# dcaustin33/intro_to_gaussian_splatting

Measured on AMD Instinct MI355X. Metric: Mpixels/sec forward raster (1M Gaussians, 1080p) + max |dpixel| vs CPU ref, higher is better.
Workload: dtype f32; 1 GPU; C3: synthetic 1M Gaussians, 1920x1080 (metric config); n_gaussians=1000000, width=1920, height=1080, tile=16, semantics=ref_cpu, layout=wh3, frames_in_flight=1, launch=one hipGraph replay per frame, frame_sync=speculative (GSX_FLAG_NO_SYNC), counts confirmed after the timed region, parallelism=1 GPU

## Files before the change

intro_to_gaussian_splatting_amd/csrc/gsx_blend.hip:

```cpp
#include <type_traits>

#include "gsx_internal.h"
#include "gsx_schedule_device.h"

namespace gsx {
namespace {

constexpr uint32_t kBatchCost = 5;
constexpr int kPad = 8, kSlots = 64 + kPad;
constexpr int kBlocks = 4;
struct __attribute__((aligned(16))) Staged {
    float4 rec[3][kSlots];
    uint16_t list[kBlocks][kSlots];
};

__device__ __forceinline__ uint32_t xcd_remap(uint32_t b, uint32_t n) {
    uint32_t xcd = b & 7u, i = b >> 3, q = n >> 3, r = n & 7u;
    uint32_t start = xcd < r ? xcd * (q + 1u) : r * (q + 1u) + (xcd - r) * q;
    return start + i;
}

__device__ __forceinline__ uint32_t scheduled_tile(uint32_t b, uint32_t nt, const uint32_t *__restrict__ sched) {
    if (!sched) return xcd_remap(b, nt);
    const uint32_t round = b >> 10, slot = b & 1023u;
    const uint32_t in_round = min(1024u, nt - (round << 10));
    return sched[(round << 10) + ((round & 1u) ? in_round - 1u - slot : slot)];
}

__device__ __forceinline__ uint32_t xcd_scheduled_tile(uint32_t b, uint32_t nt, uint32_t cap, const uint32_t *__restrict__ sched,
                                                       const uint32_t *__restrict__ header) {
    if (header[kHintSched] != nt) return b < nt ? xcd_remap(b, nt) : nt;
    const uint32_t x = b & 7u, i = b >> 3, mine = header[kHintXcdTiles + x];
    if (i >= mine) return nt;
    const uint32_t round = i >> 7, slot = i & 127u;
    const uint32_t in_round = min(128u, mine - (round << 7));
    return sched[(size_t)x * cap + (round << 7) + ((round & 1u) ? in_round - 1u - slot : slot)];
}


__device__ __forceinline__ void clear_block(uint32_t cb, const ClearPlan &cp, float *__restrict__ base) {
    int i = 0;
#pragma unroll
    for (int k = 1; k < 4; ++k) i = (k < cp.n && cb >= (uint32_t)cp.first[k]) ? k : i;
    const uint32_t per_row = (uint32_t)cp.fw[i] * 3u;
    const uint32_t total = (uint32_t)cp.rows[i] * per_row;
    const uint32_t e0 = (cb - (uint32_t)cp.first[i]) * (uint32_t)kClearFloats;
    const uint32_t e1 = min(total, e0 + (uint32_t)kClearFloats);
    float *origin = base + (int64_t)cp.s0[i] * cp.pitch + (int64_t)cp.f0[i] * 3;
    for (uint32_t e = e0 + threadIdx.x; e < e1; e += 64) {
        const uint32_t row = e / per_row, col = e - row * per_row;
        origin[(int64_t)row * cp.pitch + col] = 0.0f;
    }
}

__global__ void __launch_bounds__(64) clear_kernel(ClearPlan cp, float *__restrict__ base) {
    clear_block(blockIdx.x, cp, base);
}

constexpr float kRefOrderFlag = 2.0f;
enum { kKindSquare = 0, kKindMono = 1, kKindRefOrder = 2 };

struct Splat {
    float mx, c0, d1, h, r11, lop, cr, cg, cb, my;
    int kind;
    uint32_t blocks;
};

// ... 14 lines not shown
    }
}
__device__ __forceinline__ float exponent_y(const Splat &g, float p, float s0, float t0) {
    if (g.kind == kKindMono) {
        const float e_p = g.my - p;
        return __builtin_fmaf(e_p, __builtin_fmaf(e_p, g.r11, t0), s0);
    }
    const float w = __builtin_fmaf(-g.r11, p, t0);
    return __builtin_fmaf(-w, w, s0);
}

template <int NPX, bool WITH_REF = true>
__device__ __forceinline__ void composite(float px, const float (&e_p)[NPX], const Splat &g, float (&T)[NPX],
                                          float (&c0)[NPX], float (&c1)[NPX], float (&c2)[NPX], int blk, float ox, float oy) {
    float s0, t0;
    exponent_x(g, px, s0, t0);
    const bool kept = (g.blocks >> blk) & 1u;
    float ta[NPX], test[NPX];
#pragma unroll
    for (int j = 0; j < NPX; ++j) {
        float alpha = (WITH_REF && g.kind == kKindRefOrder)
                          ? alpha_ref(g.mx, g.c0, g.d1, g.h, g.r11, g.my, g.lop, ox + px, oy + e_p[j])
                          : __builtin_amdgcn_exp2f(exponent_y(g, e_p[j], s0, t0));
        alpha = kept ? alpha : 0.0f;
        ta[j] = T[j] * alpha;
        test[j] = T[j] - ta[j];
    }
    float m = test[0], tmin = T[0];
#pragma unroll
    for (int j = 1; j < NPX; ++j) {
        m = fminf(m, test[j]);
        tmin = fminf(tmin, T[j]);
    }
    if (__builtin_expect(__any((m < kStopRefCpu) | (tmin == 0.0f)), 0)) {
#pragma unroll
        for (int j = 0; j < NPX; ++j) {
            const bool stop = (T[j] == 0.0f) | (test[j] < kStopRefCpu);
            ta[j] = stop ? 0.0f : ta[j];
            test[j] = stop ? 0.0f : test[j];
        }
    }
#pragma unroll
    for (int j = 0; j < NPX; ++j) {
        c0[j] = __builtin_fmaf(ta[j], g.cr, c0[j]);
        c1[j] = __builtin_fmaf(ta[j], g.cg, c1[j]);
        c2[j] = __builtin_fmaf(ta[j], g.cb, c2[j]);
        T[j] = test[j];
    }
}

constexpr uint32_t kSkipBudget = 1u << 23;
enum { kBatchRegular = 0, kBatchWild = 1, kBatchMono = 2, kBatchRefOrder = 3, kBatchRefWild = 4, kBatchKindMask = 7, kBatchHasRef = 8 };
static_assert(kBatchMono < kBatchRefOrder, "the plain instances stop at kind >= kBatchRefOrder and composite a monomial-only batch");
enum { kStageWhole = 0, kStageBlocks = 1, kStageOneBlock = 2 };

__device__ __forceinline__ float skip_threshold(float bound, uint32_t &skipped, uint32_t budget) {
    const unsigned long long far1 = __ballot(bound < -26.0f), far2 = __ballot(bound < -33.0f), far3 = __ballot(bound < -40.0f);
    const uint32_t n3 = (uint32_t)__popcll(far3), n2 = (uint32_t)__popcll(far2) - n3, n1 = (uint32_t)__popcll(far1) - n2 - n3;
    const uint32_t cost3 = n3, cost23 = cost3 + (n2 << 7), cost123 = cost23 + (n1 << 14);
    if (skipped + cost123 <= budget) {
        skipped += cost123;
        return -26.0f;
    }
    if (skipped + cost23 <= budget) {
        skipped += cost23;
        return -33.0f;
    }
    if (skipped + cost3 <= budget) {
        skipped += cost3;
        return -40.0f;
    }
    return -__builtin_inff();
}

template <int MODE, bool WITH_REF = true>
__device__ __forceinline__ int stage_records(float4 a, float4 b, float4 c, bool have, uint32_t &nb, Staged &sh, int lane,
                                             float tile_x0, float tile_y0, float tile_side, uint32_t (&skipped)[kBlocks],
                                             uint32_t budget, int blk, uint32_t (&count)[kBlocks], uint32_t dead = 0u,
                                             unsigned long long *ref_slots = nullptr, const float4 *__restrict__ qraw = nullptr,
                                             uint32_t gi = 0u) {
    bool irregular = false, mono = false, refo = false;
    float bound[kBlocks] = {0.0f, 0.0f, 0.0f, 0.0f};
    float x_abs = 0.0f, y_abs = 0.0f;
    if (have) {
        refo = c.z == kRefOrderFlag;
        mono = !refo && c.z != 0.0f;
        if (WITH_REF) {
            x_abs = a.x;
            y_abs = a.y;
        }
        a.x -= tile_x0;
        a.y -= tile_y0;
        const bool bounded = !mono && a.z >= 0.0f;
        const float bx = a.x, by = a.y, bd1 = a.z, bh = a.w, br11 = b.x, blop = refo ? b.y + 0.02f : b.y;
        if (bounded) {
            auto over = [&](float x_lo, float x_hi, float y_lo, float y_hi) -> float {
                const float ex0 = bx - x_lo, ex1 = bx - x_hi;
                const float ey0 = by - y_lo, ey1 = by - y_hi;
                const float ex_min2 = ex0 * ex1 <= 0.0f ? 0.0f : fminf(ex0 * ex0, ex1 * ex1);
                const float w00 = __builtin_fmaf(br11, ey0, bh * ex0), w01 = __builtin_fmaf(br11, ey1, bh * ex0);
                const float w10 = __builtin_fmaf(br11, ey0, bh * ex1), w11 = __builtin_fmaf(br11, ey1, bh * ex1);
                const float wlo = fminf(fminf(w00, w01), fminf(w10, w11)), whi = fmaxf(fmaxf(w00, w01), fmaxf(w10, w11));
                const float wabs = fminf(fabsf(wlo), fabsf(whi));
                const float w_min2 = (wlo <= 0.0f && whi >= 0.0f) ? 0.0f : wabs * wabs;
                return blop - bd1 * ex_min2 - w_min2;
            };
            if (MODE == kStageWhole) {
                bound[0] = over(0.0f, tile_side - 1.0f, 0.0f, tile_side - 1.0f);
            } else if (MODE == kStageOneBlock) {
                bound[0] = over(8.0f * (float)(blk & 1), 8.0f * (float)(blk & 1) + 7.0f, 8.0f * (float)(blk >> 1), 8.0f * (float)(blk >> 1) + 7.0f);
            } else {
#pragma unroll
                for (int g = 0; g < kBlocks; ++g)
                    bound[g] = over(8.0f * (float)(g & 1), 8.0f * (float)(g & 1) + 7.0f, 8.0f * (float)(g >> 1), 8.0f * (float)(g >> 1) + 7.0f);
            }
            if (refo) {
                const float hi = tile_side - 1.0f;
                const float ex = fmaxf(fabsf(bx), fabsf(bx - hi)), ey = fmaxf(fabsf(by), fabsf(by - hi));
                const float S = 0.69314718f * ((bd1 + bh * bh) * (ex * ex) + 2.0f * fabsf(bh) * br11 * (ex * ey) + (br11 * br11) * (ey * ey));
                const float amax = __builtin_amdgcn_exp2f(fminf(over(0.0f, hi, 0.0f, hi), 0.0f));
                const float delta = 2.4e-7f * S;
                if (delta < 0.1f && delta * amax < 2e-5f) {
                    refo = false;
                    c.z = 0.0f;
                } else {
                    const float slack = 1.4427f * delta;
#pragma unroll
                    for (int g = 0; g < kBlocks; ++g) bound[g] += slack;
                }
            }
        }
        irregular = mono || refo || !(a.z >= 0.0f);
    }
    uint32_t bits = 0;
    unsigned long long kept_by[kBlocks] = {0ull, 0ull, 0ull, 0ull};
    if (MODE == kStageBlocks) {
#pragma unroll
        for (int g = 0; g < kBlocks; ++g) {
            if ((dead >> g) & 1u) continue;
            const float thr = skip_threshold(bound[g], skipped[g], budget);
            const bool k = have && !(bound[g] < thr);
            bits |= k ? (1u << g) : 0u;
            kept_by[g] = __ballot(k);
        }
    } else {
        const float thr = skip_threshold(bound[0], skipped[MODE == kStageOneBlock ? blk : 0], budget);
        bits = (have && !(bound[0] < thr)) ? 0xFu : 0u;
    }
    const bool keep = bits != 0u;
    float4 q4 = make_float4(0.f, 0.f, 0.f, 0.f);
    if (WITH_REF && refo && keep) q4 = qraw[gi];
    const unsigned long long mask = __ballot(keep);
    nb = (uint32_t)__popcll(mask);
    const uint32_t slot = __builtin_amdgcn_mbcnt_hi((uint32_t)(mask >> 32), __builtin_amdgcn_mbcnt_lo((uint32_t)mask, 0u));
    if (MODE == kStageBlocks) {
        const uint16_t null_slot = (uint16_t)(nb * 16u);
#pragma unroll
        for (int g = 0; g < kBlocks; ++g) {
            sh.list[g][lane] = null_slot;
            if (lane < kPad) sh.list[g][64 + lane] = null_slot;
        }
    }
    if (keep) {
        c.w = __uint_as_float(bits);
        if (WITH_REF && refo) {
            a = make_float4(x_abs, y_abs, q4.x, q4.y);
            b.x = q4.z;
            b.y = c.y;
            c.y = q4.w;
        } else {
            c.y = a.y;
            if (!mono) a.y = __builtin_fmaf(b.x, a.y, a.w * a.x);
        }
        sh.rec[0][slot] = a;
        sh.rec[1][slot] = b;
        sh.rec[2][slot] = c;
        if (MODE == kStageBlocks) {
#pragma unroll
            for (int g = 0; g < kBlocks; ++g)
                if ((bits >> g) & 1u)
                    sh.list[g][__builtin_amdgcn_mbcnt_hi((uint32_t)(kept_by[g] >> 32), __builtin_amdgcn_mbcnt_lo((uint32_t)kept_by[g], 0u))] = (uint16_t)(slot * 16u);
        }
    }
    if (MODE == kStageBlocks) {
#pragma unroll
        for (int g = 0; g < kBlocks; ++g) count[g] = (uint32_t)__popcll(kept_by[g]);
    }
    if (lane < kPad) {
        sh.rec[0][nb + lane] = make_float4(0.0f, 0.0f, 0.0f, 0.0f);
        sh.rec[1][nb + lane] = make_float4(0.0f, -__builtin_inff(), 0.0f, 0.0f);
        sh.rec[2][nb + lane] = make_float4(0.0f, 0.0f, 0.0f, __uint_as_float(0xFu));
    }
    unsigned long long ref_lanes = __ballot(refo && keep), in_slots = 0ull;
    while (ref_lanes) {
        const int l = __builtin_ctzll(ref_lanes);
        ref_lanes &= ref_lanes - 1ull;
        in_slots |= 1ull << __popcll(mask & ((1ull << l) - 1ull));
    }
    if (ref_slots) *ref_slots = in_slots;
    const int kind = (__any(mono && keep) && (WITH_REF || !in_slots))
                         ? kBatchMono
                         : (in_slots ? ((WITH_REF && __any(irregular && !refo && keep)) ? kBatchRefWild : kBatchRefOrder)
                                     : (__any(irregular && keep) ? kBatchWild : kBatchRegular));
    return kind | ((WITH_REF && in_slots) ? kBatchHasRef : 0);
}

template <int MODE, bool WITH_REF = true>
__device__ __forceinline__ int stage_batch(const Record *__restrict__ rec, const float4 *__restrict__ qraw,
                                           const uint32_t *__restrict__ vals,
                                           uint32_t base, uint32_t &nb, Staged &sh, int lane, float tile_x0,
                                           float tile_y0, float tile_side, uint32_t (&skipped)[kBlocks], uint32_t (&count)[kBlocks],
                                           uint32_t budget = kSkipBudget, const uint32_t *idx = nullptr, int blk = 0,
                                           uint32_t dead = 0u, unsigned long long *ref_slots = nullptr) {
    float4 a = make_float4(0.f, 0.f, 0.f, 0.f), b = a, c = a;
    const bool have = (uint32_t)lane < nb;
    uint32_t gi = 0u;
    if (have) {
        gi = idx ? *idx : vals[base + lane];
        const Record *q = rec + gi;
        a = q->a;
        b = q->b;
        c = q->c;
    }
    return stage_records<MODE, WITH_REF>(a, b, c, have, nb, sh, lane, tile_x0, tile_y0, tile_side, skipped, budget, blk, count, dead,
                                         ref_slots, qraw, gi);
}

typedef float v2f __attribute__((ext_vector_type(2)));

__device__ __forceinline__ v2f pk_fma(v2f a, v2f b, v2f c) { return __builtin_elementwise_fma(a, b, c); }
__device__ __forceinline__ v2f pk_exp2(v2f p) { return v2f{__builtin_amdgcn_exp2f(p.x), __builtin_amdgcn_exp2f(p.y)}; }
__device__ __forceinline__ v2f splat2(float v) { return v2f{v, v}; }

__device__ __forceinline__ void alphas(float4 A, float r11, float lop, float cx, v2f cya, v2f cyb, v2f &al_a,
                                       v2f &al_b) {
    const float e_x = A.x - cx;
    const float s0 = __builtin_fmaf(-(A.z * e_x), e_x, lop);
    const float c = __builtin_fmaf(-A.w, cx, A.y);
    const v2f wa = pk_fma(splat2(-r11), cya, splat2(c)), wb = pk_fma(splat2(-r11), cyb, splat2(c));
    al_a = pk_exp2(pk_fma(-wa, wa, splat2(s0)));
    al_b = pk_exp2(pk_fma(-wb, wb, splat2(s0)));
}

__device__ __forceinline__ void alphas_mono(float4 A, float yp, float q11, float lop, float cx, v2f cya, v2f cyb, v2f &al_a,
                                            v2f &al_b) {
    const float e_x = A.x - cx;
    const float s0 = __builtin_fmaf(e_x * e_x, A.z, lop);
    const float t0 = e_x * A.w;
    const v2f ea = splat2(yp) - cya, eb = splat2(yp) - cyb;
    al_a = pk_exp2(pk_fma(ea, pk_fma(ea, splat2(q11), splat2(t0)), splat2(s0)));
    al_b = pk_exp2(pk_fma(eb, pk_fma(eb, splat2(q11), splat2(t0)), splat2(s0)));
}

__device__ __forceinline__ void alphas_ref(float4 A, float q10, float q11, float op, float fx, v2f fya, v2f fyb, v2f &al_a,
                                           v2f &al_b) {
    const float e0 = A.x - fx, d0 = -0.5f * e0;
    const float p00 = d0 * A.z, p01 = d0 * A.w;
    const v2f e1a = splat2(A.y) - fya, e1b = splat2(A.y) - fyb;
    const v2f d1a = splat2(-0.5f) * e1a, d1b = splat2(-0.5f) * e1b;
    const v2f t0a = pk_fma(d1a, splat2(q10), splat2(p00)), t0b = pk_fma(d1b, splat2(q10), splat2(p00));
    const v2f t1a = pk_fma(d1a, splat2(q11), splat2(p01)), t1b = pk_fma(d1b, splat2(q11), splat2(p01));
    const v2f pa = t0a * splat2(e0) + t1a * e1a, pb = t0b * splat2(e0) + t1b * e1b;
    const float l2e = 1.44269504088896340736f;
    al_a = pk_exp2(pa * splat2(l2e)) * splat2(op);
    al_b = pk_exp2(pb * splat2(l2e)) * splat2(op);
}

#define GSX_ACCUMULATE(ta_a, ta_b, cr, cg, cb)          \
    do {                                                \
        c0a = pk_fma(ta_a, splat2(cr), c0a);            \
        c1a = pk_fma(ta_a, splat2(cg), c1a);            \
        c2a = pk_fma(ta_a, splat2(cb), c2a);            \
        c0b = pk_fma(ta_b, splat2(cr), c0b);            \
        c1b = pk_fma(ta_b, splat2(cg), c1b);            \
        c2b = pk_fma(ta_b, splat2(cb), c2b);            \
    } while (0)

__device__ __forceinline__ void checked_pair(v2f alpha, v2f &T, v2f &ta) {
// ... 127 lines not shown
                    const float w = __builtin_fmaf(-Bq.x, cy, __builtin_fmaf(-A.w, cx, A.y));
                    alpha[u] = __builtin_amdgcn_exp2f(__builtin_fmaf(-w, w, s0));
                }
                float ta[kTrip], Tt = T;
                if (!checked) {
                    float m = T;
#pragma unroll
                    for (int u = 0; u < kTrip; ++u) {
                        ta[u] = Tt * alpha[u];
                        Tt = Tt - ta[u];
                        m = fminf(m, Tt);
                    }
                    if (__builtin_expect(__any(!(m >= kStopRefCpu)), 0)) {
                        checked = true;
                        Tt = T;
                    }
                }
                if (checked) {
#pragma unroll
                    for (int u = 0; u < kTrip; ++u) {
                        const float t_a = Tt * alpha[u], t = Tt - t_a;
                        const bool stop = (Tt == 0.0f) | (t < kStopRefCpu);
                        ta[u] = stop ? 0.0f : t_a;
                        Tt = stop ? 0.0f : t;
                    }
                }
#pragma unroll
                for (int u = 0; u < kTrip; ++u) {
                    const float2 rg_ = *reinterpret_cast<const float2 *>(&sh.rec[1][k + u].z);
                    const float cb = sh.rec[2][k + u].x;
                    c0 = __builtin_fmaf(ta[u], rg_.x, c0);
                    c1 = __builtin_fmaf(ta[u], rg_.y, c1);
                    c2 = __builtin_fmaf(ta[u], cb, c2);
                }
                T = Tt;
            }
        }
        tile_sync<REF>();
        if (__ballot(T > 0.0f) == 0ull) break;
    }
    if (cost_out && lane == 0) atomicMax(cost_out, cost | 0x80000000u);
    if (REF && saw_ref && lane == 0 && redo) atomicAdd(redo, 1u);
    float *o = out.ptr + (int64_t)(px - out.x0) * out.stride_x + (int64_t)(py - out.y0) * out.stride_y;
    o[0] = c0;
    o[1] = c1;
    o[2] = c2;
}

template <bool REF>
__device__ __forceinline__ void blend_tile16(const Record *__restrict__ rec, const float4 *__restrict__ qraw,
                                             const uint32_t *__restrict__ vals,
                                             const uint2 *__restrict__ ranges, const TileGrid &g, const OutDesc &out,
                                             const LongTiles &lt, uint32_t budget, const BlendHints &hints, const TileSpan &span,
                                             uint32_t t, Staged &sh) {
    const int lane = REF ? (int)(threadIdx.x & 63u) : (int)threadIdx.x;
    const int tx = g.wx0 + (int)(t / (uint32_t)g.nwy()), ty = g.wy0 + (int)(t % (uint32_t)g.nwy());
    if ((span.axis ? ty : tx) < span.lo || (span.axis ? ty : tx) >= span.hi) return;
    const bool y_contig = out.stride_y < out.stride_x;
    const int lx = y_contig ? (lane >> 2) : (lane & 15);
    const int ly0 = 4 * (y_contig ? (lane & 3) : (lane >> 4));
    const int px = tx * 16 + lx, py0 = ty * 16 + ly0;
    const float cx = (float)lx;
    float cy[4];
#pragma unroll
    for (int j = 0; j < 4; ++j) cy[j] = (float)(ly0 + j);
    const v2f cya = v2f{cy[0], cy[1]}, cyb = v2f{cy[2], cy[3]};
    const int blk = (lx >> 3) | ((ly0 >> 3) << 1);
    const uint16_t *my_list = sh.list[blk];
    const char *rec_a = reinterpret_cast<const char *>(&sh.rec[0][0]), *rec_b = reinterpret_cast<const char *>(&sh.rec[1][0]),
               *rec_c = reinterpret_cast<const char *>(&sh.rec[2][0]);

    float T[4] = {1.0f, 1.0f, 1.0f, 1.0f};
    float c0[4] = {0, 0, 0, 0}, c1[4] = {0, 0, 0, 0}, c2[4] = {0, 0, 0, 0};
    v2f Ta = splat2(1.0f), Tb = splat2(1.0f);
    v2f c0a = splat2(0.0f), c1a = c0a, c2a = c0a, c0b = c0a, c1b = c0a, c2b = c0a;

    bool checked = false;
    bool restart_scalar = false;
    uint2 rg = ranges[t];
    rg.x = (uint32_t)__builtin_amdgcn_readfirstlane((int)rg.x);
    rg.y = (uint32_t)__builtin_amdgcn_readfirstlane((int)rg.y);
    if (hints.lens && lane == 0 && t == 0) {
        const bool by_cost = hints.header[kHintLens] == (uint32_t)g.count() && hints.header[kHintSched] == (uint32_t)g.count();
        hints.header[kHintLens] = (uint32_t)g.count();
        if (lt.max && by_cost) {
            const uint32_t found = *lt.count, pct = max(hints.header[kHintLongPct], lt.cost_pct);
            hints.header[kHintLongPct] = found > 192u ? min(pct + pct / 4u, 1000u) : (found < 64u ? max(pct - pct / 8u, lt.cost_pct) : pct);
        }
    }
    if (rg.y & kLongFlag) return;
    bool saw_ref = false;
    uint32_t cost = 0;
    uint32_t skipped[kBlocks] = {0u, 0u, 0u, 0u};
    unsigned long long lanes_of[kBlocks];
#pragma unroll
    for (int gb = 0; gb < kBlocks; ++gb) lanes_of[gb] = __ballot(blk == gb);
    uint32_t dead = 0u;
    uint32_t idx = rg.x + (uint32_t)lane < rg.y ? vals[rg.x + lane] : 0u;
    for (uint32_t base = rg.x; base < rg.y; base += 64) {
        uint32_t nb = (uint32_t)__builtin_amdgcn_readfirstlane((int)min(64u, rg.y - base));
        const uint32_t idx_now = idx;
        if (base + 64u + (uint32_t)lane < rg.y) idx = vals[base + 64u + lane];
        uint32_t count[kBlocks];
        unsigned long long ref_slots = 0ull;
        const int kind_all = stage_batch<kStageBlocks, REF>(rec, qraw, vals, base, nb, sh, lane, (float)(tx * 16), (float)(ty * 16),
                                                            16.0f, skipped, count, budget, &idx_now, 0, dead, &ref_slots);
        const int kind = kind_all & kBatchKindMask;
        const bool wild = kind != kBatchRegular;
        if (REF && (kind_all & kBatchHasRef)) saw_ref = true;
        const uint32_t nl = max(max(count[0], count[1]), max(count[2], count[3]));
        cost += nl + kBatchCost;
        tile_sync<REF>();
        if (!REF && kind >= kBatchRefOrder) {
            if (lane == 0) atomicAdd(lt.redo, 1u);
            return;
        } else if (kind == kBatchMono) {
            restart_scalar = true;
            break;
        } else {
            constexpr int kTrip = 4;
            uint32_t k = 0;
            auto trip = [&](auto n_tag) __attribute__((always_inline)) -> bool {
                constexpr int N = decltype(n_tag)::value;
                v2f ta_a[N], ta_b[N], ta = Ta, tb = Tb;
                uint32_t slot[N];
#pragma unroll
                for (int u = 0; u < N; ++u) {
                    slot[u] = my_list[k + u];
                    const float4 A = *reinterpret_cast<const float4 *>(rec_a + slot[u]);
                    const float2 Bq = *reinterpret_cast<const float2 *>(rec_b + slot[u]);
                    v2f aa, ab;
                    alphas(A, Bq.x, Bq.y, cx, cya, cyb, aa, ab);
                    ta_a[u] = ta * aa;
                    ta_b[u] = tb * ab;
                    ta = ta - ta_a[u];
                    tb = tb - ta_b[u];
                }
                if (__builtin_expect(__any(!(min4(ta, tb) >= kStopRefCpu)), 0)) return false;
#pragma unroll
                for (int u = 0; u < N; ++u) {
                    const float2 rg_ = *reinterpret_cast<const float2 *>(rec_b + slot[u] + 8);
                    const float cb = *reinterpret_cast<const float *>(rec_c + slot[u]);
                    GSX_ACCUMULATE(ta_a[u], ta_b[u], rg_.x, rg_.y, cb);
                }
                Ta = ta;
                Tb = tb;
                k += N;
                return true;
            };
            auto exact_pair = [&]() __attribute__((always_inline)) {
                const uint32_t s0_ = my_list[k], s1_ = my_list[k + 1];
// ... 9 lines not shown
                checked_pair(aa1, Ta, ta1a);
                checked_pair(ab1, Tb, ta1b);
                GSX_ACCUMULATE(ta1a, ta1b, B1.z, B1.w, cb1);
                k += 2;
            };
            if (!wild) {
                while (!checked && k + kTrip <= nl) checked = !trip(std::integral_constant<int, kTrip>());
                while (!checked && k < nl) checked = !trip(std::integral_constant<int, 2>());
            }
            if (!REF || kind < kBatchRefOrder) {
                while (k < nl) exact_pair();
            } else {
                const float fx_ = (float)(tx * 16) + cx;
                const v2f fya = splat2((float)(ty * 16)) + cya, fyb = splat2((float)(ty * 16)) + cyb;
                auto is_ref = [&](uint32_t s_) -> bool { return (s_ >> 4) < 64u && ((ref_slots >> (s_ >> 4)) & 1ull) != 0ull; };
                while (k < nl) {
                    if (kind == kBatchRefOrder && !checked && k + kTrip <= nl) {
                        bool flagged = false;
#pragma unroll
                        for (int u = 0; u < kTrip; ++u) flagged |= is_ref(my_list[k + u]);
                        if (!__any(flagged)) {
                            checked = !trip(std::integral_constant<int, kTrip>());
                            continue;
                        }
                    }
                    const uint32_t s0_ = my_list[k], s1_ = my_list[k + 1];
                    const bool r0 = is_ref(s0_), r1 = is_ref(s1_);
                    if (!__any(r0 | r1)) {
                        exact_pair();
                        continue;
                    }
                    const float4 A0 = *reinterpret_cast<const float4 *>(rec_a + s0_), B0 = *reinterpret_cast<const float4 *>(rec_b + s0_);
                    const float2 C0 = *reinterpret_cast<const float2 *>(rec_c + s0_);
                    v2f aa, ab, ta_a, ta_b;
                    if (r0)
                        alphas_ref(A0, B0.x, C0.y, B0.y, fx_, fya, fyb, aa, ab);
                    else
                        alphas(A0, B0.x, B0.y, cx, cya, cyb, aa, ab);
                    checked_pair(aa, Ta, ta_a);
                    checked_pair(ab, Tb, ta_b);
                    GSX_ACCUMULATE(ta_a, ta_b, B0.z, B0.w, C0.x);
                    k += 1;
                }
            }
        }
        tile_sync<REF>();
        const unsigned long long alive = __ballot((Ta.x > 0.0f) | (Ta.y > 0.0f) | (Tb.x > 0.0f) | (Tb.y > 0.0f));
        if (alive == 0ull) break;
        if (checked) {
#pragma unroll
            for (int gb = 0; gb < kBlocks; ++gb) dead |= (alive & lanes_of[gb]) == 0ull ? (1u << gb) : 0u;
        }
    }
    if (restart_scalar) {
        tile_sync<REF>();
#pragma unroll
        for (int j = 0; j < 4; ++j) {
            T[j] = 1.0f;
            c0[j] = c1[j] = c2[j] = 0.0f;
        }
#pragma unroll
        for (int gb = 0; gb < kBlocks; ++gb) skipped[gb] = 0u;
        for (uint32_t base = rg.x; base < rg.y; base += 64) {
            uint32_t nb = (uint32_t)__builtin_amdgcn_readfirstlane((int)min(64u, rg.y - base));
            uint32_t count[kBlocks];
            const int later = stage_batch<kStageBlocks, REF>(rec, qraw, vals, base, nb, sh, lane, (float)(tx * 16), (float)(ty * 16),
                                                             16.0f, skipped, count, budget);
            if (REF && (later & kBatchHasRef)) saw_ref = true;
            if (!REF && (later & kBatchKindMask) >= kBatchRefOrder) {
                if (lane == 0) atomicAdd(lt.redo, 1u);
                return;
            }
            cost += 4u * nb;
            tile_sync<REF>();
            for (uint32_t k = 0; k < nb; ++k) {
                const Splat s = read_splat(sh, k);
                composite<4, REF>(cx, cy, s, T, c0, c1, c2, blk, (float)(tx * 16), (float)(ty * 16));
            }
            tile_sync<REF>();
            if (__ballot((T[0] > 0.0f) | (T[1] > 0.0f) | (T[2] > 0.0f) | (T[3] > 0.0f)) == 0ull) break;
        }
    } else {
        c0[0] = c0a.x; c0[1] = c0a.y; c0[2] = c0b.x; c0[3] = c0b.y;
        c1[0] = c1a.x; c1[1] = c1a.y; c1[2] = c1b.x; c1[3] = c1b.y;
        c2[0] = c2a.x; c2[1] = c2a.y; c2[2] = c2b.x; c2[3] = c2b.y;
    }

    if (hints.lens && lane == 0) hints.lens[t] = cost;
    if (REF && saw_ref && lane == 0 && lt.redo) atomicAdd(lt.redo, 1u);
    float *o = out.ptr + (int64_t)(px - out.x0) * out.stride_x + (int64_t)(py0 - out.y0) * out.stride_y;
    if (y_contig && (reinterpret_cast<uintptr_t>(o) & 15u) == 0) {
        float4 *o4 = reinterpret_cast<float4 *>(o);
        o4[0] = make_float4(c0[0], c1[0], c2[0], c0[1]);
        o4[1] = make_float4(c1[1], c2[1], c0[2], c1[2]);
        o4[2] = make_float4(c2[2], c0[3], c1[3], c2[3]);
    } else {
#pragma unroll
        for (int j = 0; j < 4; ++j) {
            float *oj = o + (int64_t)j * out.stride_y;
            oj[0] = c0[j];
            oj[1] = c1[j];
            oj[2] = c2[j];
        }
    }
}

template <bool REF>
__device__ __forceinline__ void blend_tile16_grid(const Record *__restrict__ rec, const float4 *__restrict__ qraw,
                                                  const uint32_t *__restrict__ vals, const uint2 *__restrict__ ranges,
                                                  const TileGrid &g, const OutDesc &out, const ClearPlan &cp, const LongTiles &lt,
                                                  uint32_t nhelpers, const uint32_t *__restrict__ sched, uint32_t budget,
                                                  const BlendHints &hints, uint32_t tile_blocks, uint32_t sched_cap_,
                                                  const TileSpan &span, Staged &sh) {
    const uint32_t nrank = hints.samples ? kRankGroups : 0u;
    const uint32_t rank0 = hints.rank_last ? gridDim.x - nrank : 0u;
    if (blockIdx.x - rank0 < nrank) {
        if (span.first) rank_samples(blockIdx.x - rank0, (int)threadIdx.x, hints);
        return;
    }
    const uint32_t block = hints.rank_last ? blockIdx.x : blockIdx.x - nrank;
    if (block < nhelpers) {
        const uint32_t b = block, slot = (b >> 5) * 8u + (b & 7u);
        const int quarter = (int)((b >> 3) & 3u);
        if (slot >= min(*lt.count, lt.max)) return;
        const uint32_t lt_tile = lt.list[slot];
        {
            const int lead = span.axis ? g.wy0 + (int)(lt_tile % (uint32_t)g.nwy()) : g.wx0 + (int)(lt_tile / (uint32_t)g.nwy());
            if (lead < span.lo || lead >= span.hi) return;
        }
        blend_long_tile_quarter<REF>(rec, qraw, vals, ranges, g, out, lt_tile, quarter, sh, budget,
                                     hints.lens ? hints.lens + lt_tile : nullptr, lt.redo);
        return;
    }
    const uint32_t bid = block - nhelpers;
    if (bid >= tile_blocks) {
        if (span.first) clear_block(bid - tile_blocks, cp, out.ptr);
        return;
    }
    const uint32_t t = hints.xcd_sched ? xcd_scheduled_tile(bid, (uint32_t)g.count(), sched_cap_, sched, hints.header)
                                       : scheduled_tile(bid, (uint32_t)g.count(), sched);
    if (t >= (uint32_t)g.count()) return;
    blend_tile16<REF>(rec, qraw, vals, ranges, g, out, lt, budget, hints, span, t, sh);
}

#ifndef GSX_PLAIN_WAVES
#define GSX_PLAIN_WAVES 8
#endif
__global__ void __launch_bounds__(64) __attribute__((amdgpu_waves_per_eu(GSX_PLAIN_WAVES, 8)))
    blend_tile16_kernel(const Record *__restrict__ rec, const float4 *__restrict__ qraw, const uint32_t *__restrict__ vals,
                        const uint2 *__restrict__ ranges, TileGrid g, OutDesc out, ClearPlan cp, LongTiles lt,
                        uint32_t nhelpers, const uint32_t *__restrict__ sched, uint32_t budget, BlendHints hints,
                        uint32_t tile_blocks, uint32_t sched_cap_, TileSpan span) {
    __shared__ Staged sh;
    blend_tile16_grid<false>(rec, qraw, vals, ranges, g, out, cp, lt, nhelpers, sched, budget, hints, tile_blocks, sched_cap_, span, sh);
}

#ifndef GSX_REF_WAVES
#define GSX_REF_WAVES 4
#endif
__global__ void __launch_bounds__(64) __attribute__((amdgpu_waves_per_eu(GSX_REF_WAVES, 8)))
    blend_tile16_ref_kernel(const Record *__restrict__ rec, const float4 *__restrict__ qraw, const uint32_t *__restrict__ vals,
                            const uint2 *__restrict__ ranges, TileGrid g, OutDesc out, ClearPlan cp, LongTiles lt,
                            uint32_t nhelpers, const uint32_t *__restrict__ sched, uint32_t budget, BlendHints hints,
                            uint32_t tile_blocks, uint32_t sched_cap_, TileSpan span) {
    __shared__ Staged sh;
    blend_tile16_grid<true>(rec, qraw, vals, ranges, g, out, cp, lt, nhelpers, sched, budget, hints, tile_blocks, sched_cap_, span, sh);
}

__global__ void __launch_bounds__(64)
    blend_generic_kernel(const Record *__restrict__ rec, const float4 *__restrict__ qraw, const uint32_t *__restrict__ vals,
                         const uint2 *__restrict__ ranges, TileGrid g, OutDesc out, ClearPlan cp) {
    __shared__ Staged sh;
    if (blockIdx.x >= (uint32_t)g.count()) {
        clear_block(blockIdx.x - (uint32_t)g.count(), cp, out.ptr);
        return;
    }
    const int lane = threadIdx.x;
    const uint32_t t = xcd_remap(blockIdx.x, (uint32_t)g.count());
    const int tx = g.wx0 + (int)(t / (uint32_t)g.nwy()), ty = g.wy0 + (int)(t % (uint32_t)g.nwy());
    const int Ts = g.tile, npx = Ts * Ts;
    const uint2 rg = ranges[t];
    const bool fast_y = out.stride_y < out.stride_x;
    const bool blocks = Ts == 16;
    for (int chunk = 0; chunk < npx; chunk += 64) {
        uint32_t skipped[kBlocks] = {0u, 0u, 0u, 0u}, count[kBlocks];
        const int p = chunk + lane;
        const bool valid = p < npx;
        const int pf = p % Ts, ps = p / Ts;
        const int lx = fast_y ? ps : pf, ly = fast_y ? pf : ps;
        const int px = tx * Ts + lx, py = ty * Ts + ly;
        const float fx = (float)lx, fy = (float)ly;
        const int blk = blocks ? ((lx >> 3) | ((ly >> 3) << 1)) & 3 : 0;
        float T[1] = {1.0f}, c0[1] = {0.0f}, c1[1] = {0.0f}, c2[1] = {0.0f};
        for (uint32_t base = rg.x; base < rg.y; base += 64) {
            uint32_t nb = min(64u, rg.y - base);
            if (blocks)
                (void)stage_batch<kStageBlocks>(rec, qraw, vals, base, nb, sh, lane, (float)(tx * Ts), (float)(ty * Ts), (float)Ts, skipped, count);
            else
                (void)stage_batch<kStageWhole>(rec, qraw, vals, base, nb, sh, lane, (float)(tx * Ts), (float)(ty * Ts), (float)Ts, skipped, count);
            __syncthreads();
            for (uint32_t k = 0; k < nb; ++k) {
                const Splat s = read_splat(sh, k);
                const float e_p[1] = {fy};
                composite<1>(fx, e_p, s, T, c0, c1, c2, blk, (float)(tx * Ts), (float)(ty * Ts));
            }
            __syncthreads();
            if (__ballot(valid && T[0] > 0.0f) == 0ull) break;
        }
        if (valid) {
            float *o = out.ptr + (int64_t)(px - out.x0) * out.stride_x + (int64_t)(py - out.y0) * out.stride_y;
            o[0] = c0[0];
            o[1] = c1[0];
            o[2] = c2[0];
        }
    }
}

constexpr float kStdAlphaMin = 1.0f / 255.0f, kStdStop = 0.0001f;
// ... 314 lines not shown
```

intro_to_gaussian_splatting_amd/gaussian_scene.py:

```python
from __future__ import annotations

import ctypes
from collections import OrderedDict
from typing import Dict, Optional, Sequence, Tuple

import torch

from . import _ffi
from .colmap import read_camera_file, read_image_file
from .gaussians import Gaussians
from .image import GaussianImage
from .schema import PreprocessedScene


def _ptr(t: Optional[torch.Tensor]):
    return ctypes.c_void_p(0 if t is None else t.data_ptr())


def _check_f32(name: str, t: torch.Tensor, device: torch.device) -> torch.Tensor:
    if t.dtype != torch.float32:
        raise TypeError("%s must be float32, got %s" % (name, t.dtype))
    if t.device != device:
        raise ValueError("%s is on %s, expected %s" % (name, t.device, device))
    return t if t.is_contiguous() else t.contiguous()
# ... 578 lines not shown
            dev = g.points.device
            _require_gpu(dev)
            n = int(g.points.shape[0])
            k = (int(g.sh_degree) + 1) ** 2
            pts = _check_f32("points", g.points.detach().reshape(n, 3), dev)
            sh = _check_f32("sh", g.sh.detach().reshape(n, k, 3), dev)
            gc = _check_f32("grad_colors", grad_colors.detach().reshape(n, 3), dev)
            gsh = torch.empty((n, k, 3), dtype=torch.float32, device=dev)
            gview = torch.empty((n, 3), dtype=torch.float32, device=dev) if with_points else None
            center = (ctypes.c_float * 3)(*self.images[image_idx].camera_center_host)
            with torch.cuda.device(dev):
                rc = lib.gsx_sh_backward(_ptr(pts), _ptr(sh), int(g.sh_degree), n, center, _ptr(gc), _ptr(gsh), _ptr(gview),
                                         _stream_handle(dev))
            _ffi.check(rc)
        return gsh, gview

    def _note_count(self, cap_key, n_instances: int, n_kept: int = 0, n_redo: Optional[int] = None) -> None:
        self._instances_hint = max(self._instances_hint, int(n_instances * 1.1))
        self._cap_hints[cap_key] = int(n_instances * 1.1) + 4096
        self._kept_hints[cap_key] = max(1, int(n_kept))
        if n_redo is not None:
            self._n_redo_seen[cap_key] = int(n_redo)
        if cap_key[2] is None and cap_key[3] == "ref_cpu":
            self._last_instances = n_instances

    def _ensure_pinned_pool(self) -> None:
        if self._pinned_pool is None:
            self._pinned_pool = torch.zeros((_PINNED_SLOTS, ctypes.sizeof(_ffi.GsxFrameStats)),
                                            dtype=torch.uint8).pin_memory()

    def _pinned_slot(self) -> torch.Tensor:
        self._ensure_pinned_pool()
        slot = self._pinned_pool[self._pinned_next % _PINNED_SLOTS]
        self._pinned_next += 1
        slot.zero_()
        return slot

    def confirm_frames(self) -> int:
        if not self._pending:
            return 0
        torch.cuda.synchronize(self.gaussians.points.device)
        redone = 0
        pending, self._pending = self._pending, []
        for pinned, cap_key, ran_plain, call in pending:
            st = ctypes.cast(ctypes.c_void_p(pinned.data_ptr()), ctypes.POINTER(_ffi.GsxFrameStats)).contents
            self._note_count(cap_key, int(st.n_instances), int(st.n_kept), int(st.n_redo))
            if st.n_instances > st.reserved or (ran_plain and st.n_redo > 0):
                redone += 1
                self.render_image_hip(**call)
        return redone

    def capture_frame(self, image_idx: int, tile_size: int = 16, layout: str = "wh3",
                      semantics: str = "ref_cpu", movable_camera: bool = False,
                      headroom: float = 1.1) -> "CapturedFrame":
        if _wants_grad(self.gaussians):
            _refuse_with_grad("capture_frame")
        dev = self.gaussians.points.device
        _require_gpu(dev)
        cam = self.images[image_idx].gsx_camera()
        shape = (cam.width, cam.height, 3) if layout == "wh3" else (cam.height, cam.width, 3)
        out = torch.empty(shape, dtype=torch.float32, device=dev)
        cam_buf = None
        if movable_camera:
            cam_buf = torch.frombuffer(bytearray(bytes(cam)), dtype=torch.uint8).to(dev)
        kw = dict(tile_size=tile_size, layout=layout, out=out, semantics=semantics, camera_buffer=cam_buf)
        st = {}
        self.render_image_hip(image_idx, stats=st, **kw)
        lib = _ffi.load()
        n = int(self.gaussians.points.shape[0])
        cap = int(st["n_instances"] * max(float(headroom), 1.0)) + 4096
        nbytes = lib.gsx_workspace_bytes(n, cam.width, cam.height, tile_size, cap)
        if nbytes == 0:
            raise _ffi.GsxError(_ffi.GSX_ERR_INVALID_ARGUMENT, "gsx_workspace_bytes rejected the sizes")
        private = dict(cap=cap, workspace=torch.empty(nbytes, dtype=torch.uint8, device=dev), kept=int(st["n_kept"]),
                       rows_flag=0 if semantics == "std_3dgs" else _ffi.rows_flag(n, int(st["n_visible"])),
                       plain=(not movable_camera) and int(st.get("n_redo", 1)) == 0 and
                       int(st.get("n_tiles", 0)) >= _PLAIN_MIN_TILES,
                       pinned=torch.zeros(ctypes.sizeof(_ffi.GsxFrameStats), dtype=torch.uint8).pin_memory(), inputs=[],
                       hints=[torch.zeros(lib.gsx_hints_bytes(cam.width, cam.height, tile_size), dtype=torch.uint8,
                                          device=dev), False])
        stream = torch.cuda.Stream(dev)
        with torch.cuda.stream(stream):
            self.render_image_hip(image_idx, _private=private, **kw)
        torch.cuda.synchronize(dev)
        graph = torch.cuda.CUDAGraph()
        with torch.cuda.graph(graph, stream=stream):
            self.render_image_hip(image_idx, no_sync=True, _private=private, **kw)
        call = dict(image_idx=image_idx, **kw)
        frame = CapturedFrame(self, graph, out, private["pinned"], call, camera_buffer=cam_buf,
                              workspace=private["workspace"], capacity=cap, inputs=private["inputs"])
        frame._hints = private["hints"][0]
        frame._plain_footprints = bool(private["plain"])
        return frame

    def render_image(self, image_idx: int, tile_size: int = 16, geometry_gradients: bool = False) -> torch.Tensor:
        frame = self.render_image_hip(image_idx, tile_size=tile_size, layout="wh3", geometry_gradients=geometry_gradients)
        host = torch.empty(frame.shape, dtype=frame.dtype, pin_memory=True)
        host.copy_(frame, non_blocking=True)
        torch.cuda.current_stream(frame.device).synchronize()
        return host

    render = render_image

    def render_images(self, image_indices, tile_size: int = 16):
        if _wants_grad(self.gaussians):
            _refuse_with_grad("render_images")
        dev = self.gaussians.points.device
        _require_gpu(dev)
        copy_stream = torch.cuda.Stream(dev)
        frames, hosts, copied, checks, pending = [None, None], [None, None], [None, None], [None, None], None

        def finish(k: int) -> torch.Tensor:
            copied[k].synchronize()
            if checks[k] is not None:
                pinned, cap_key, ran_plain, call = checks[k]
                st = ctypes.cast(ctypes.c_void_p(pinned.data_ptr()), ctypes.POINTER(_ffi.GsxFrameStats)).contents
                self._note_count(cap_key, int(st.n_instances), int(st.n_kept), int(st.n_redo))
                if st.n_instances > st.reserved or (ran_plain and st.n_redo > 0):
# ... 64 lines not shown
```

Measured before the change: 6031 Mpixels/s.

## Add run-ahead double-buffered ring staging to the ref_cpu tile blend kernel

Replaces the per-batch staged list in the REF blend path with a double-buffered record area and a per-block circular index ring. The wave can stage the next 64-record batch while blocks still have queued entries from the previous one, cutting the sync-per-batch stall and letting sub-blocks advance unevenly. It also raises the waves-per-EU hint from 4 to 5, recomputes the output pixel addressing from the lane id, and adds a split_long_tiles option to capture_frame. The cost is more complex control flow, extra LDS per workgroup, and higher register pressure.

```diff
diff --git a/intro_to_gaussian_splatting_amd/csrc/gsx_blend.hip b/intro_to_gaussian_splatting_amd/csrc/gsx_blend.hip
--- a/intro_to_gaussian_splatting_amd/csrc/gsx_blend.hip
+++ b/intro_to_gaussian_splatting_amd/csrc/gsx_blend.hip
@@ -13,6 +13,13 @@
     float4 rec[3][kSlots];
     uint16_t list[kBlocks][kSlots];
 };
+
+constexpr int kRing = 256, kTripPad = 4, kNullSlot = 2 * 64;
+struct __attribute__((aligned(16))) RunAhead {
+    float4 rec[3][kNullSlot + 1];
+    uint16_t ring[kRing + 2 * kTripPad][kBlocks];
+};
+static_assert(sizeof(RunAhead) >= sizeof(Staged) && sizeof(RunAhead) <= 10240, "160 KiB of LDS per CU / 16 workgroups");
 
 __device__ __forceinline__ uint32_t xcd_remap(uint32_t b, uint32_t n) {
     uint32_t xcd = b & 7u, i = b >> 3, q = n >> 3, r = n & 7u;
@@ -133,7 +140,7 @@
 constexpr uint32_t kSkipBudget = 1u << 23;
 enum { kBatchRegular = 0, kBatchWild = 1, kBatchMono = 2, kBatchRefOrder = 3, kBatchRefWild = 4, kBatchKindMask = 7, kBatchHasRef = 8 };
 static_assert(kBatchMono < kBatchRefOrder, "the plain instances stop at kind >= kBatchRefOrder and composite a monomial-only batch");
-enum { kStageWhole = 0, kStageBlocks = 1, kStageOneBlock = 2 };
+enum { kStageWhole = 0, kStageBlocks = 1, kStageOneBlock = 2, kStageRing = 3 };
 
 __device__ __forceinline__ float skip_threshold(float bound, uint32_t &skipped, uint32_t budget) {
     const unsigned long long far1 = __ballot(bound < -26.0f), far2 = __ballot(bound < -33.0f), far3 = __ballot(bound < -40.0f);
@@ -154,12 +161,13 @@
     return -__builtin_inff();
 }
 
-template <int MODE, bool WITH_REF = true>
-__device__ __forceinline__ int stage_records(float4 a, float4 b, float4 c, bool have, uint32_t &nb, Staged &sh, int lane,
+template <int MODE, bool WITH_REF = true, class SH = Staged>
+__device__ __forceinline__ int stage_records(float4 a, float4 b, float4 c, bool have, uint32_t &nb, SH &sh, int lane,
                                              float tile_x0, float tile_y0, float tile_side, uint32_t (&skipped)[kBlocks],
                                              uint32_t budget, int blk, uint32_t (&count)[kBlocks], uint32_t dead = 0u,
                                              unsigned long long *ref_slots = nullptr, const float4 *__restrict__ qraw = nullptr,
-                                             uint32_t gi = 0u) {
+                                             uint32_t gi = 0u, uint32_t buf = 0u, const uint32_t *wr = nullptr) {
+    constexpr bool kPerBlock = MODE == kStageBlocks || MODE == kStageRing;
     bool irregular = false, mono = false, refo = false;
     float bound[kBlocks] = {0.0f, 0.0f, 0.0f, 0.0f};
     float x_abs = 0.0f, y_abs = 0.0f;
@@ -215,7 +223,7 @@
     }
     uint32_t bits = 0;
     unsigned long long kept_by[kBlocks] = {0ull, 0ull, 0ull, 0ull};
-    if (MODE == kStageBlocks) {
+    if (kPerBlock) {
 #pragma unroll
         for (int g = 0; g < kBlocks; ++g) {
             if ((dead >> g) & 1u) continue;
@@ -233,8 +241,9 @@
     if (WITH_REF && refo && keep) q4 = qraw[gi];
     const unsigned long long mask = __ballot(keep);
     nb = (uint32_t)__popcll(mask);
-    const uint32_t slot = __builtin_amdgcn_mbcnt_hi((uint32_t)(mask >> 32), __builtin_amdgcn_mbcnt_lo((uint32_t)mask, 0u));
-    if (MODE == kStageBlocks) {
+    const uint32_t slot = (MODE == kStageRing ? buf * 64u : 0u) +
+                          __builtin_amdgcn_mbcnt_hi((uint32_t)(mask >> 32), __builtin_amdgcn_mbcnt_lo((uint32_t)mask, 0u));
+    if constexpr (MODE == kStageBlocks) {
         const uint16_t null_slot = (uint16_t)(nb * 16u);
 #pragma unroll
         for (int g = 0; g < kBlocks; ++g) {
@@ -256,18 +265,35 @@
         sh.rec[0][slot] = a;
         sh.rec[1][slot] = b;
         sh.rec[2][slot] = c;
-        if (MODE == kStageBlocks) {
+        if constexpr (MODE == kStageBlocks) {
 #pragma unroll
             for (int g = 0; g < kBlocks; ++g)
                 if ((bits >> g) & 1u)
                     sh.list[g][__builtin_amdgcn_mbcnt_hi((uint32_t)(kept_by[g] >> 32), __builtin_amdgcn_mbcnt_lo((uint32_t)kept_by[g], 0u))] = (uint16_t)(slot * 16u);
         }
-    }
-    if (MODE == kStageBlocks) {
+        if constexpr (MODE == kStageRing) {
+#pragma unroll
+            for (int g = 0; g < kBlocks; ++g)
+                if ((bits >> g) & 1u) {
+                    const uint32_t at = (wr[g] + __builtin_amdgcn_mbcnt_hi((uint32_t)(kept_by[g] >> 32), __builtin_amdgcn_mbcnt_lo((uint32_t)kept_by[g], 0u))) & (uint32_t)(kRing - 1);
+                    sh.ring[at][g] = (uint16_t)(slot * 16u);
+                    if (at < (uint32_t)kTripPad) sh.ring[kRing + at][g] = (uint16_t)(slot * 16u);
+                }
+        }
+    }
+    if (kPerBlock) {
 #pragma unroll
         for (int g = 0; g < kBlocks; ++g) count[g] = (uint32_t)__popcll(kept_by[g]);
     }
-    if (lane < kPad) {
+    if constexpr (MODE == kStageRing) {
+        if (lane < kBlocks * kTripPad) {
+            const int g = lane / kTripPad;
+            const uint32_t end = g == 0 ? wr[0] + count[0] : (g == 1 ? wr[1] + count[1] : (g == 2 ? wr[2] + count[2] : wr[3] + count[3]));
+            const uint32_t at = (end + (uint32_t)(lane % kTripPad)) & (uint32_t)(kRing - 1);
+            sh.ring[at][g] = (uint16_t)(kNullSlot * 16);
+            if (at < (uint32_t)kTripPad) sh.ring[kRing + at][g] = (uint16_t)(kNullSlot * 16);
+        }
+    } else if (lane < kPad) {
         sh.rec[0][nb + lane] = make_float4(0.0f, 0.0f, 0.0f, 0.0f);
         sh.rec[1][nb + lane] = make_float4(0.0f, -__builtin_inff(), 0.0f, 0.0f);
         sh.rec[2][nb + lane] = make_float4(0.0f, 0.0f, 0.0f, __uint_as_float(0xFu));
@@ -286,13 +312,14 @@
     return kind | ((WITH_REF && in_slots) ? kBatchHasRef : 0);
 }
 
-template <int MODE, bool WITH_REF = true>
+template <int MODE, bool WITH_REF = true, class SH = Staged>
 __device__ __forceinline__ int stage_batch(const Record *__restrict__ rec, const float4 *__restrict__ qraw,
                                            const uint32_t *__restrict__ vals,
-                                           uint32_t base, uint32_t &nb, Staged &sh, int lane, float tile_x0,
+                                           uint32_t base, uint32_t &nb, SH &sh, int lane, float tile_x0,
                                            float tile_y0, float tile_side, uint32_t (&skipped)[kBlocks], uint32_t (&count)[kBlocks],
                                            uint32_t budget = kSkipBudget, const uint32_t *idx = nullptr, int blk = 0,
-                                           uint32_t dead = 0u, unsigned long long *ref_slots = nullptr) {
+                                           uint32_t dead = 0u, unsigned long long *ref_slots = nullptr, uint32_t buf = 0u,
+                                           const uint32_t *wr = nullptr) {
     float4 a = make_float4(0.f, 0.f, 0.f, 0.f), b = a, c = a;
     const bool have = (uint32_t)lane < nb;
     uint32_t gi = 0u;
@@ -303,8 +330,8 @@
         b = q->b;
         c = q->c;
     }
-    return stage_records<MODE, WITH_REF>(a, b, c, have, nb, sh, lane, tile_x0, tile_y0, tile_side, skipped, budget, blk, count, dead,
-                                         ref_slots, qraw, gi);
+    return stage_records<MODE, WITH_REF, SH>(a, b, c, have, nb, sh, lane, tile_x0, tile_y0, tile_side, skipped, budget, blk, count, dead,
+                                             ref_slots, qraw, gi, buf, wr);
 }
 
 typedef float v2f __attribute__((ext_vector_type(2)));
@@ -538,7 +565,8 @@
                                              const uint32_t *__restrict__ vals,
                                              const uint2 *__restrict__ ranges, const TileGrid &g, const OutDesc &out,
                                              const LongTiles &lt, uint32_t budget, const BlendHints &hints, const TileSpan &span,
-                                             uint32_t t, Staged &sh) {
+                                             uint32_t t, std::conditional_t<REF, RunAhead, Staged> &sh_all) {
+    Staged &sh = reinterpret_cast<Staged &>(sh_all);
     const int lane = REF ? (int)(threadIdx.x & 63u) : (int)threadIdx.x;
     const int tx = g.wx0 + (int)(t / (uint32_t)g.nwy()), ty = g.wy0 + (int)(t % (uint32_t)g.nwy());
     if ((span.axis ? ty : tx) < span.lo || (span.axis ? ty : tx) >= span.hi) return;
@@ -552,9 +580,8 @@
     for (int j = 0; j < 4; ++j) cy[j] = (float)(ly0 + j);
     const v2f cya = v2f{cy[0], cy[1]}, cyb = v2f{cy[2], cy[3]};
     const int blk = (lx >> 3) | ((ly0 >> 3) << 1);
-    const uint16_t *my_list = sh.list[blk];
-    const char *rec_a = reinterpret_cast<const char *>(&sh.rec[0][0]), *rec_b = reinterpret_cast<const char *>(&sh.rec[1][0]),
-               *rec_c = reinterpret_cast<const char *>(&sh.rec[2][0]);
+    const char *rec_a = reinterpret_cast<const char *>(&sh_all.rec[0][0]), *rec_b = reinterpret_cast<const char *>(&sh_all.rec[1][0]),
+               *rec_c = reinterpret_cast<const char *>(&sh_all.rec[2][0]);
 
     float T[4] = {1.0f, 1.0f, 1.0f, 1.0f};
     float c0[4] = {0, 0, 0, 0}, c1[4] = {0, 0, 0, 0}, c2[4] = {0, 0, 0, 0};
@@ -583,6 +610,202 @@
     for (int gb = 0; gb < kBlocks; ++gb) lanes_of[gb] = __ballot(blk == gb);
     uint32_t dead = 0u;
     uint32_t idx = rg.x + (uint32_t)lane < rg.y ? vals[rg.x + lane] : 0u;
+    if constexpr (REF) {
+        const char *ring = reinterpret_cast<const char *>(&sh_all.ring[0][0]);
+        constexpr uint32_t kRingWrap = (uint32_t)(kRing * kBlocks * sizeof(uint16_t)) - 1u;
+        if (lane == 0) {
+            sh_all.rec[0][kNullSlot] = make_float4(0.0f, 0.0f, 0.0f, 0.0f);
+            sh_all.rec[1][kNullSlot] = make_float4(0.0f, -__builtin_inff(), 0.0f, 0.0f);
+            sh_all.rec[2][kNullSlot] = make_float4(0.0f, 0.0f, 0.0f, __uint_as_float(0xFu));
+        }
+        const uint32_t nbatch = (rg.y - rg.x + 63u) >> 6;
+        uint32_t staged = 0u;
+        uint32_t wr[kBlocks] = {0u, 0u, 0u, 0u}, end_older[kBlocks] = {0u, 0u, 0u, 0u};
+        uint32_t rp = 2u * (uint32_t)blk, queued = 0u;
+        unsigned long long ref_mask[2] = {0ull, 0ull};
+        int buf_kind[2] = {kBatchRegular, kBatchRegular};
+        auto trip = [&](auto n_tag) __attribute__((always_inline)) -> bool {
+            constexpr int N = decltype(n_tag)::value;
+            const uint16_t *e = reinterpret_cast<const uint16_t *>(ring + (rp & kRingWrap));
+            v2f ta_a[N], ta_b[N], ta = Ta, tb = Tb;
+            uint32_t slot[N];
+#pragma unroll
+            for (int u = 0; u < N; ++u) {
+                slot[u] = e[u * kBlocks];
+                const float4 A = *reinterpret_cast<const float4 *>(rec_a + slot[u]);
+                const float2 Bq = *reinterpret_cast<const float2 *>(rec_b + slot[u]);
+                v2f aa, ab;
+                alphas(A, Bq.x, Bq.y, cx, cya, cyb, aa, ab);
+                ta_a[u] = ta * aa;
+                ta_b[u] = tb * ab;
+                ta = ta - ta_a[u];
+                tb = tb - ta_b[u];
+            }
+            if (__builtin_expect(__any(!(min4(ta, tb) >= kStopRefCpu)), 0)) return false;
+#pragma unroll
+            for (int u = 0; u < N; ++u) {
+                const float2 rg_ = *reinterpret_cast<const float2 *>(rec_b + slot[u] + 8);
+                const float cb = *reinterpret_cast<const float *>(rec_c + slot[u]);
+                GSX_ACCUMULATE(ta_a[u], ta_b[u], rg_.x, rg_.y, cb);
+            }
+            Ta = ta;
+            Tb = tb;
+            const uint32_t step = min((uint32_t)N, queued);
+            queued -= step;
+            rp += 8u * step;
+            return true;
+        };
+        auto exact_pair = [&]() __attribute__((always_inline)) {
+            const uint16_t *e = reinterpret_cast<const uint16_t *>(ring + (rp & kRingWrap));
+            const uint32_t s0_ = e[0], s1_ = e[kBlocks];
+            const float4 A0 = *reinterpret_cast<const float4 *>(rec_a + s0_), B0 = *reinterpret_cast<const float4 *>(rec_b + s0_);
+            const float4 A1 = *reinterpret_cast<const float4 *>(rec_a + s1_), B1 = *reinterpret_cast<const float4 *>(rec_b + s1_);
+            const float cb0 = *reinterpret_cast<const float *>(rec_c + s0_), cb1 = *reinterpret_cast<const float *>(rec_c + s1_);
+            v2f aa0, ab0, aa1, ab1, ta0a, ta0b, ta1a, ta1b;
+            alphas(A0, B0.x, B0.y, cx, cya, cyb, aa0, ab0);
+            alphas(A1, B1.x, B1.y, cx, cya, cyb, aa1, ab1);
+            checked_pair(aa0, Ta, ta0a);
+            checked_pair(ab0, Tb, ta0b);
+            GSX_ACCUMULATE(ta0a, ta0b, B0.z, B0.w, cb0);
+            checked_pair(aa1, Ta, ta1a);
+            checked_pair(ab1, Tb, ta1b);
+            GSX_ACCUMULATE(ta1a, ta1b, B1.z, B1.w, cb1);
+            const uint32_t step = min(2u, queued);
+            queued -= step;
+            rp += 8u * step;
+        };
+        auto is_ref = [&](uint32_t s_) -> bool {
+            const uint32_t i_ = s_ >> 4;
+            return i_ < (uint32_t)kNullSlot && (((i_ & 64u) ? ref_mask[1] : ref_mask[0]) >> (i_ & 63u)) & 1ull;
+        };
+        for (;;) {
+            uint32_t least = 0xFFFFFFFFu, most = 0u;
+            bool older_done = true;
+            const bool more = staged < nbatch;
+#pragma unroll
+            for (int gb = 0; gb < kBlocks; ++gb) {
+                const uint32_t q = (uint32_t)__builtin_amdgcn_readlane((int)queued, __builtin_ctzll(lanes_of[gb]));
+                if (q != 0u || (more && !((dead >> gb) & 1u))) least = min(least, q);
+                most = max(most, q);
+                older_done = older_done && q <= wr[gb] - end_older[gb];
+            }
+            unsigned long long alive = ~0ull;
+            if (checked) {
+                alive = __ballot((Ta.x > 0.0f) | (Ta.y > 0.0f) | (Tb.x > 0.0f) | (Tb.y > 0.0f));
+                if (alive == 0ull) break;
+            }
+            if (more && (staged < 2u || (least < (uint32_t)kTripPad && older_done))) {
+#ifdef GSX_TEST_HOOKS
+                {
+                    const uint32_t newer = blk == 0 ? wr[0] - end_older[0] : (blk == 1 ? wr[1] - end_older[1] : (blk == 2 ? wr[2] - end_older[2] : wr[3] - end_older[3]));
+                    if (staged >= 2u && __any(queued > newer)) __builtin_trap();
+                }
+#endif
+                if (checked) {
+                    uint32_t died = 0u;
+#pragma unroll
+                    for (int gb = 0; gb < kBlocks; ++gb) died |= (alive & lanes_of[gb]) == 0ull ? (1u << gb) : 0u;
+                    dead |= died;
+                    if ((dead >> blk) & 1u) {
+                        rp += 8u * queued;
+                        queued = 0u;
+                    }
+                }
+                const uint32_t base = rg.x + (staged << 6), b_ = staged & 1u;
+                uint32_t nb = (uint32_t)__builtin_amdgcn_readfirstlane((int)min(64u, rg.y - base));
+                const uint32_t idx_now = idx;
+                if (base + 64u + (uint32_t)lane < rg.y) idx = vals[base + 64u + lane];
+                uint32_t count[kBlocks];
+                unsigned long long in_slots = 0ull;
+                tile_sync<true>();
+                const int kind_all = stage_batch<kStageRing, true, RunAhead>(rec, qraw, vals, base, nb, sh_all, lane, (float)(tx * 16), (float)(ty * 16),
+                                                                             16.0f, skipped, count, budget, &idx_now, 0, dead, &in_slots, b_, wr);
+                tile_sync<true>();
+                if (b_) ref_mask[1] = in_slots; else ref_mask[0] = in_slots;
+                if (kind_all & kBatchHasRef) saw_ref = true;
+                cost += kBatchCost;
+                if ((kind_all & kBatchKindMask) == kBatchMono) {
+                    restart_scalar = true;
+                    break;
+                }
+                if (b_) buf_kind[1] = kind_all & kBatchKindMask; else buf_kind[0] = kind_all & kBatchKindMask;
+#pragma unroll
+                for (int gb = 0; gb < kBlocks; ++gb) {
+                    end_older[gb] = wr[gb];
+                    wr[gb] += count[gb];
+                }
+                queued += blk == 0 ? count[0] : (blk == 1 ? count[1] : (blk == 2 ? count[2] : count[3]));
+                ++staged;
+                continue;
+            }
+            if (most == 0u) break;
+            int left = !more ? (int)most : (least >= (uint32_t)kTripPad ? (int)(least & ~(uint32_t)(kTripPad - 1)) : kTripPad);
+            const int k_old = (older_done || staged < 2u) ? (int)kBatchRegular : ((staged & 1u) ? buf_kind[1] : buf_kind[0]);
+            const int k_new = (staged & 1u) ? buf_kind[0] : buf_kind[1];
+            const bool any_ref = k_old >= kBatchRefOrder || k_new >= kBatchRefOrder;
+            const bool any_wild = k_old == kBatchWild || k_old == kBatchRefWild || k_new == kBatchWild || k_new == kBatchRefWild;
+            if (!any_ref && !any_wild) {
+                while (!checked && left > 0) {
+                    checked = !trip(std::integral_constant<int, 4>());
+                    if (!checked) {
+                        left -= 4;
+                        cost += 4u;
+                    }
+                }
+            }
+            if (!any_ref) {
+                while (left > 0) {
+                    exact_pair();
+                    left -= 2;
+                    cost += 2u;
+                }
+            } else {
+                const float fx_ = (float)(tx * 16) + cx;
+                const v2f fya = splat2((float)(ty * 16)) + cya, fyb = splat2((float)(ty * 16)) + cyb;
+                while (left > 0) {
+                    if (!any_wild && !checked && left >= 4) {
+                        const uint16_t *e = reinterpret_cast<const uint16_t *>(ring + (rp & kRingWrap));
+                        bool flagged = false;
+#pragma unroll
+                        for (int u = 0; u < 4; ++u) flagged |= is_ref(e[u * kBlocks]);
+                        if (!__any(flagged)) {
+                            checked = !trip(std::integral_constant<int, 4>());
+                            if (!checked) {
+                                left -= 4;
+                                cost += 4u;
+                            }
+                            continue;
+                        }
+                    }
+                    const uint16_t *e = reinterpret_cast<const uint16_t *>(ring + (rp & kRingWrap));
+                    const uint32_t s0_ = e[0], s1_ = e[kBlocks];
+                    const bool r0 = is_ref(s0_), r1 = is_ref(s1_);
+                    if (!__any(r0 | r1)) {
+                        exact_pair();
+                        left -= 2;
+                        cost += 2u;
+                        continue;
+                    }
+                    const float4 A0 = *reinterpret_cast<const float4 *>(rec_a + s0_), B0 = *reinterpret_cast<const float4 *>(rec_b + s0_);
+                    const float2 C0 = *reinterpret_cast<const float2 *>(rec_c + s0_);
+                    v2f aa, ab, ta_a, ta_b;
+                    if (r0)
+                        alphas_ref(A0, B0.x, C0.y, B0.y, fx_, fya, fyb, aa, ab);
+                    else
+                        alphas(A0, B0.x, B0.y, cx, cya, cyb, aa, ab);
+                    checked_pair(aa, Ta, ta_a);
+                    checked_pair(ab, Tb, ta_b);
+                    GSX_ACCUMULATE(ta_a, ta_b, B0.z, B0.w, C0.x);
+                    const uint32_t step = min(1u, queued);
+                    queued -= step;
+                    rp += 8u * step;
+                    left -= 1;
+                    cost += 1u;
+                }
+            }
+        }
+    } else {
+    const uint16_t *my_list = sh.list[blk];
     for (uint32_t base = rg.x; base < rg.y; base += 64) {
         uint32_t nb = (uint32_t)__builtin_amdgcn_readfirstlane((int)min(64u, rg.y - base));
         const uint32_t idx_now = idx;
@@ -698,6 +921,7 @@
             for (int gb = 0; gb < kBlocks; ++gb) dead |= (alive & lanes_of[gb]) == 0ull ? (1u << gb) : 0u;
         }
     }
+    }
     if (restart_scalar) {
         tile_sync<REF>();
 #pragma unroll
@@ -734,7 +958,13 @@
 
     if (hints.lens && lane == 0) hints.lens[t] = cost;
     if (REF && saw_ref && lane == 0 && lt.redo) atomicAdd(lt.redo, 1u);
-    float *o = out.ptr + (int64_t)(px - out.x0) * out.stride_x + (int64_t)(py0 - out.y0) * out.stride_y;
+    int px_ = px, py0_ = py0;
+    if constexpr (REF) {
+        const int l_ = (int)__builtin_amdgcn_mbcnt_hi(~0u, __builtin_amdgcn_mbcnt_lo(~0u, 0u));
+        px_ = tx * 16 + (y_contig ? (l_ >> 2) : (l_ & 15));
+        py0_ = ty * 16 + 4 * (y_contig ? (l_ & 3) : (l_ >> 4));
+    }
+    float *o = out.ptr + (int64_t)(px_ - out.x0) * out.stride_x + (int64_t)(py0_ - out.y0) * out.stride_y;
     if (y_contig && (reinterpret_cast<uintptr_t>(o) & 15u) == 0) {
         float4 *o4 = reinterpret_cast<float4 *>(o);
         o4[0] = make_float4(c0[0], c1[0], c2[0], c0[1]);
@@ -757,7 +987,7 @@
                                                   const TileGrid &g, const OutDesc &out, const ClearPlan &cp, const LongTiles &lt,
                                                   uint32_t nhelpers, const uint32_t *__restrict__ sched, uint32_t budget,
                                                   const BlendHints &hints, uint32_t tile_blocks, uint32_t sched_cap_,
-                                                  const TileSpan &span, Staged &sh) {
+                                                  const TileSpan &span, std::conditional_t<REF, RunAhead, Staged> &sh) {
     const uint32_t nrank = hints.samples ? kRankGroups : 0u;
     const uint32_t rank0 = hints.rank_last ? gridDim.x - nrank : 0u;
     if (blockIdx.x - rank0 < nrank) {
@@ -774,7 +1004,7 @@
             const int lead = span.axis ? g.wy0 + (int)(lt_tile % (uint32_t)g.nwy()) : g.wx0 + (int)(lt_tile / (uint32_t)g.nwy());
             if (lead < span.lo || lead >= span.hi) return;
         }
-        blend_long_tile_quarter<REF>(rec, qraw, vals, ranges, g, out, lt_tile, quarter, sh, budget,
+        blend_long_tile_quarter<REF>(rec, qraw, vals, ranges, g, out, lt_tile, quarter, reinterpret_cast<Staged &>(sh), budget,
                                      hints.lens ? hints.lens + lt_tile : nullptr, lt.redo);
         return;
     }
@@ -802,14 +1032,14 @@
 }
 
 #ifndef GSX_REF_WAVES
-#define GSX_REF_WAVES 4
+#define GSX_REF_WAVES 5
 #endif
 __global__ void __launch_bounds__(64) __attribute__((amdgpu_waves_per_eu(GSX_REF_WAVES, 8)))
     blend_tile16_ref_kernel(const Record *__restrict__ rec, const float4 *__restrict__ qraw, const uint32_t *__restrict__ vals,
                             const uint2 *__restrict__ ranges, TileGrid g, OutDesc out, ClearPlan cp, LongTiles lt,
                             uint32_t nhelpers, const uint32_t *__restrict__ sched, uint32_t budget, BlendHints hints,
                             uint32_t tile_blocks, uint32_t sched_cap_, TileSpan span) {
-    __shared__ Staged sh;
+    __shared__ RunAhead sh;
     blend_tile16_grid<true>(rec, qraw, vals, ranges, g, out, cp, lt, nhelpers, sched, budget, hints, tile_blocks, sched_cap_, span, sh);
 }
 
diff --git a/intro_to_gaussian_splatting_amd/gaussian_scene.py b/intro_to_gaussian_splatting_amd/gaussian_scene.py
--- a/intro_to_gaussian_splatting_amd/gaussian_scene.py
+++ b/intro_to_gaussian_splatting_amd/gaussian_scene.py
@@ -654,7 +654,7 @@
 
     def capture_frame(self, image_idx: int, tile_size: int = 16, layout: str = "wh3",
                       semantics: str = "ref_cpu", movable_camera: bool = False,
-                      headroom: float = 1.1) -> "CapturedFrame":
+                      headroom: float = 1.1, split_long_tiles: bool = True) -> "CapturedFrame":
         if _wants_grad(self.gaussians):
             _refuse_with_grad("capture_frame")
         dev = self.gaussians.points.device
@@ -666,6 +666,8 @@
         if movable_camera:
             cam_buf = torch.frombuffer(bytearray(bytes(cam)), dtype=torch.uint8).to(dev)
         kw = dict(tile_size=tile_size, layout=layout, out=out, semantics=semantics, camera_buffer=cam_buf)
+        if not split_long_tiles:
+            kw["split_long_tiles"] = False
         st = {}
         self.render_image_hip(image_idx, stats=st, **kw)
         lib = _ffi.load()
```

After: 5618 Mpixels/s. 0.931x the previous value.
